# burmajam/delta_crdt_ex

Hardware: AMD Instinct MI355X
Metric: merged dots/sec for AWLWWMap delta join + Merkle diff keys/sec at 1–8 GPUs (higher is better)
Workload: dtype u64; 1 GPU; config2: 1M-key AWLWWMap full-state join of two replicas, 10% concurrent-write conflicts, per GPU (key-hash range shards); keys_per_gpu=1000000, rows_in_per_gpu=2000000, rows_out_per_gpu=1100011, parallelism=key-hash shards x1, rotate=4

## Files before the change

delta_crdt_ex_amd/csrc/api_engine.hip:

```cpp
#include <mutex>

#include <chrono>
#include <cstdarg>
#include <cstdio>
#include <cstdlib>

#include "dg_engine.h"

struct DevShare {
  int engines = 0;
  hipStream_t stream = nullptr;
};
std::mutex g_share_mu;
DevShare g_share[64];

hipStream_t shared_join_stream(dg_engine* e) {
  std::lock_guard<std::mutex> g(g_share_mu);
  DevShare& d = g_share[e->device & 63];
  if (d.engines < 2) return nullptr;
  if (!d.stream && hipStreamCreateWithFlags(&d.stream, hipStreamNonBlocking) != hipSuccess)
    d.stream = nullptr;
  return d.stream;
}

// ... 152 lines not shown
}

int check_store(const dg_store* s, const char* what) {
  if (!s) return fail(DG_E_INVAL, "%s: null store", what);
  if (s->n && (!s->key || !s->val || !s->ts || !s->node || !s->cnt))
    return fail(DG_E_INVAL, "%s: null column with n=%llu", what, (unsigned long long)s->n);
  return DG_OK;
}

int check_ctx(const dg_context* c, const char* what) {
  if (!c) return fail(DG_E_INVAL, "%s: null context", what);
  if (c->kind != DG_CTX_VV && c->kind != DG_CTX_DOTS)
    return fail(DG_E_INVAL, "%s: bad context kind %d", what, c->kind);
  if (c->n && (!c->node || !c->cnt)) return fail(DG_E_INVAL, "%s: null context column", what);
  return DG_OK;
}

bool pair_aligned(const void* k, const void* v, const void* t, const void* n, const void* c) {
  return !(((uintptr_t)k | (uintptr_t)v | (uintptr_t)t | (uintptr_t)c) & 15) && !((uintptr_t)n & 7);
}

int settle(dg_engine* e) {
  if (!e->pending.empty()) return dg_engine_sync(e);
  return DG_OK;
}

MerkleT merkle_of(const dg_merkle* t) {
  MerkleT m;
  m.depth = t->depth;
  m.sb = t->shard_bits;
  m.shard = t->shard;
  m.nodes = t->nodes;
  m.counts = t->counts;
  m.th = TermH{};
  if (t->terms) {
    m.th.nh = t->terms->node_hash;
    m.th.nn = t->terms->node_hash ? t->terms->n_nodes : 0;
    m.th.vid = t->terms->val_id;
    m.th.vh = t->terms->val_hash;
    m.th.nv = (t->terms->val_id && t->terms->val_hash) ? t->terms->n_vals : 0;
    m.th.on = 1;
  }
  m.starts = t->starts;
  return m;
}

int check_merkle(const dg_merkle* t, const char* what) {
  if (!t || !t->nodes) return fail(DG_E_INVAL, "%s: null tree", what);
  if (!t->counts || ((uintptr_t)t->counts & 15))
    return fail(DG_E_INVAL, "%s: the tree's counts must be a 16-byte aligned device array", what);
  if (t->depth < 1 || t->depth > 28) return fail(DG_E_INVAL, "%s: depth %u not in 1..28", what, t->depth);
  if (t->shard_bits > 16 || t->depth + t->shard_bits > 44)
    return fail(DG_E_INVAL, "%s: shard_bits %u (depth %u)", what, t->shard_bits, t->depth);
  if (t->shard_bits ? (t->shard >> t->shard_bits) != 0 : t->shard != 0)
    return fail(DG_E_INVAL, "%s: shard %llu >= 2^%u", what, (unsigned long long)t->shard, t->shard_bits);
  return DG_OK;
}

int tree_input_error(u32 bits, const char* what, const char* holds) {
  if (bits & MERKLE_ERR_SHARD) return fail(DG_E_INVAL, "%s: a key outside the tree's shard", what);
  if (bits & MERKLE_ERR_COUNT)
    return fail(DG_E_CAPACITY, "%s: a bucket %s more than 65535 rows (use a deeper tree)", what, holds);
  return DG_OK;
}

extern "C" {

int dg_abi_version(void) { return DG_ABI_VERSION; }

const char* dg_last_error(void) { return g_err.c_str(); }

int dg_engine_create(int device, void* hip_stream, dg_engine** out) {
  if (!out) return fail(DG_E_INVAL, "dg_engine_create: null out");
  *out = nullptr;
  int ndev = 0;
  HIP_TRY(hipGetDeviceCount(&ndev));
  if (device < 0 || device >= ndev)
    return fail(DG_E_INVAL, "dg_engine_create: device %d of %d", device, ndev);
  dg_engine* e = new dg_engine();
  e->device = device;
  {
    const char* v = getenv("DG_JOIN_WORKERS");
    if (v && atoi(v) > 0) e->join_workers = atoi(v);
    const char* m = getenv("DG_JOIN_MODE");
    if (m && m[0] == '2') e->join_mode = JOIN_TWO_PASS;
    const char* sp = getenv("DG_SPLICE");
    if (sp && sp[0] == '0') e->splice = false;
    const char* kd = getenv("DG_KD");
    if (kd && kd[0] == '0') e->kd = false;
    const char* am = getenv("DG_APPLY_MODE");
    if (am && strcmp(am, "fold") == 0) e->apply_mode = 1;
    if (am && strcmp(am, "onepass") == 0) e->apply_mode = 2;
    const char* tr = getenv("DG_TREE_REBUILD");
    if (tr && strcmp(tr, "always") == 0) e->tree_rebuild = dg_engine::TREE_ALWAYS;
    if (tr && strcmp(tr, "never") == 0) e->tree_rebuild = dg_engine::TREE_NEVER;
    if (tr && atoll(tr) > 0) e->tree_rebuild_div = (u64)atoll(tr);
  }
  int rc = set_device(e);
  if (rc != DG_OK) {
    delete e;
    return rc;
  }
  if (hip_stream) {
    e->stream = (hipStream_t)hip_stream;
  } else {
    if (hipStreamCreateWithFlags(&e->stream, hipStreamNonBlocking) != hipSuccess) {
      delete e;
      return fail(DG_E_DEVICE, "hipStreamCreate failed");
    }
    e->own_stream = true;
  }
  if (hipMalloc(&e->d_counts, 8 * sizeof(u64) + 16 * sizeof(u32)) != hipSuccess ||
      hipMalloc(&e->started, JOIN_MAX_GRID * sizeof(u32)) != hipSuccess ||
      hipHostMalloc(&e->h_counts, 16 * sizeof(u64), 0) != hipSuccess ||
      hipHostMalloc(&e->h_pub, 24 * sizeof(u64), hipHostMallocMapped | hipHostMallocCoherent) !=
          hipSuccess ||
      hipHostGetDevicePointer((void**)&e->d_pub, e->h_pub, 0) != hipSuccess) {
    dg_engine_destroy(e);
    return fail(DG_E_NOMEM, "dg_engine_create: allocation failed");
  }
  e->ticket = (u32*)(e->d_counts + 8);
  memset(e->h_pub, 0, 24 * sizeof(u64));
  if (hipMemsetAsync(e->d_counts, 0, 8 * sizeof(u64) + 16 * sizeof(u32), e->stream) != hipSuccess ||
      hipMemsetAsync(e->started, 0, JOIN_MAX_GRID * sizeof(u32), e->stream) != hipSuccess) {
    dg_engine_destroy(e);
    return fail(DG_E_DEVICE, "dg_engine_create: hipMemsetAsync failed");
  }
  rc = ensure_state(e, 4096);
  if (rc != DG_OK) {
    dg_engine_destroy(e);
    return rc;
  }
  if (hipEventCreateWithFlags(&e->ev_in, hipEventDisableTiming) != hipSuccess ||
      hipEventCreateWithFlags(&e->ev_out, hipEventDisableTiming) != hipSuccess) {
    dg_engine_destroy(e);
    return fail(DG_E_DEVICE, "dg_engine_create: hipEventCreate failed");
  }
  {
    std::lock_guard<std::mutex> g(g_share_mu);
    const int n = ++g_share[device & 63].engines;
    if (n == 2) hipDeviceSynchronize();
  }
  *out = e;
  return DG_OK;
}

int dg_engine_destroy(dg_engine* e) {
  if (!e) return DG_OK;
  hipSetDevice(e->device);
  if (e->stream) hipStreamSynchronize(e->stream);
  for (Buf* b : {&e->state, &e->tmp, &e->counts, &e->fold, &e->spl, &e->ubuf, &e->sml, &e->kdb, &e->kdz, &e->rpl,
                 &e->diff_bsum})
    if (b->p) hipFree(b->p);
  if (e->d_counts) hipFree(e->d_counts);
  if (e->h_counts) hipHostFree(e->h_counts);
  if (e->h_pub) hipHostFree(e->h_pub);
  if (e->started) hipFree(e->started);
  if (e->h_stage.p) hipHostFree(e->h_stage.p);
  if (e->h_cont.p) hipHostFree(e->h_cont.p);
  if (e->own_stream && e->stream) hipStreamDestroy(e->stream);
  if (e->ev_in || e->ev_out) {
    if (e->ev_in) hipEventDestroy(e->ev_in);
    if (e->ev_out) hipEventDestroy(e->ev_out);
    std::lock_guard<std::mutex> g(g_share_mu);
    DevShare& d = g_share[e->device & 63];
    if (e->ev_out && --d.engines == 0 && d.stream) {
// ... 58 lines not shown
```

delta_crdt_ex_amd/csrc/api_join.hip:

```cpp
#include "dg_engine.h"

int join2_enqueue(dg_engine* e, const dg_store* a, const dg_context* ca, const dg_store* b,
                  const dg_context* cb, const uint64_t* keys, uint64_t n_keys, dg_store* out,
                  dg_context* out_ctx, uint64_t* d_counts, void** chg, bool force_two_pass) {
  TRY(check_store(a, "dg_join2 a"));
  TRY(check_store(b, "dg_join2 b"));
  TRY(check_ctx(ca, "dg_join2 ca"));
  TRY(check_ctx(cb, "dg_join2 cb"));
  if (!out || !out_ctx || !d_counts) return fail(DG_E_INVAL, "dg_join2: null output");
  if (keys == nullptr && n_keys != 0) return fail(DG_E_INVAL, "dg_join2: keys NULL with n_keys>0");
  if (out->cap < a->n + b->n)
    return fail(DG_E_CAPACITY, "dg_join2: out cap %llu < %llu rows in", (unsigned long long)out->cap,
                (unsigned long long)(a->n + b->n));
  if (out_ctx->cap < ca->n + cb->n)
    return fail(DG_E_CAPACITY, "dg_join2: out_ctx cap %llu < %llu", (unsigned long long)out_ctx->cap,
                (unsigned long long)(ca->n + cb->n));
  if (a->n + b->n && (!out->key || !out->val || !out->ts || !out->node || !out->cnt))
    return fail(DG_E_INVAL, "dg_join2: null output column");
  TRY(set_device(e));
  const u64 tiles = join2_tiles(a->n, b->n), tiles_cap = join2_tiles_cap(a->n, b->n);
  Arena state;
  join_state_layout(state, tiles_cap);
  TRY(ensure_state(e, state.off / sizeof(u64)));
  const bool two_pass = (force_two_pass || e->join_mode == JOIN_TWO_PASS) && !chg;
  if (!two_pass) TRY(ensure_counts(e, tiles_cap));
  JoinScratch js;
  TRY(carve(e, &e->tmp, [&](Arena& m) {
    return join_layout(m, ctx_union_tmp_bytes(ca->n, cb->n),
                       two_pass ? measured([&](Arena& x) { pass_layout(x, tiles, JOIN_TILE); }) : 0,
                       chg ? measured([&](Arena& x) { chg_layout(x, tiles, JOIN_TILE); }) : 0);
  }, &js));
  if (chg) *chg = js.chg;
  Scan sc;
  TRY(next_scan(e, &sc));
  hipStream_t st = e->stream;
  hipStream_t ps = two_pass ? nullptr : shared_join_stream(e);
  if (ps) {
    HIP_TRY(hipEventRecord(e->ev_in, e->stream));
    HIP_TRY(hipStreamWaitEvent(ps, e->ev_in, 0));
    st = ps;
  }
  HIP_TRY(launch_join2(rows_of(a), ctx_of(ca), rows_of(b), ctx_of(cb), keys, keys ? n_keys : 0,
                       rows_out_of(out), out_ctx->node, out_ctx->cnt, js.ctx, js.pass,
                       two_pass ? JOIN_TWO_PASS : JOIN_SINGLE_PASS, sc, e->join_workers, d_counts, st, js.chg));
  if (ps) {
    HIP_TRY(hipEventRecord(e->ev_out, ps));
    HIP_TRY(hipStreamWaitEvent(e->stream, e->ev_out, 0));
  }
  out_ctx->kind = (ca->kind == DG_CTX_DOTS && cb->kind == DG_CTX_DOTS) ? DG_CTX_DOTS : DG_CTX_VV;
  return DG_OK;
}

bool splice_wanted(const dg_engine* e, const dg_store* a, const dg_store* b, const uint64_t* keys,
                   uint64_t n_keys, const dg_store* out) {
  return e->splice && keys && n_keys > 0 && (n_keys + b->n) * 8 <= a->n && out &&
         pair_aligned(a->key, a->val, a->ts, a->node, a->cnt) &&
         pair_aligned(out->key, out->val, out->ts, out->node, out->cnt);
}

int splice_take(dg_engine* e, const dg_store* a, const dg_store* b, const uint64_t* keys,
                uint64_t n_keys, u64 uctx_cap, Splice* w, bool* ok) {
  *ok = false;
  const u64 cap_k = std::min<u64>(a->n, 16 * n_keys + 4096);
  const u64 cap_e = cap_k + b->n;
  SpliceScratch s;
  TRY(carve(e, &e->spl, [&](Arena& m) { return splice_layout(m, cap_k, cap_e, n_keys, splice_tiles(a->n), uctx_cap); },
            &s));
  w->ak = s.ak;
  w->ed = s.ed;
  w->uctx = s.uctx;
  SpliceArgs& sp = w->sp;
  sp = SpliceArgs{};
  sp.a_lo = s.idx.a_lo;
  sp.a_off = s.idx.a_off;
  sp.end = s.idx.end;
  sp.shift = s.idx.shift;
  sp.gap = s.idx.gap;
  sp.tile_u0 = s.tile_u0;
  sp.moved = (u32*)(e->d_counts + SC_MOVED);
  TRY(ensure_state(e, take_tiles(n_keys) + 2));
  Scan sc;
  TRY(next_scan(e, &sc));
  static_assert(SC_BAD == SC_TAKEN + 1 && SC_MOVED == SC_TAKEN + 2, "zeroed as one range");
  HIP_TRY(hipMemsetAsync(e->d_counts + SC_TAKEN, 0, 3 * sizeof(u64), e->stream));
  u32* pre_len = nullptr;
  if (n_keys * 60 >= a->n) {
    pre_len = (u32*)sp.end;
    HIP_TRY(launch_splice_locate(rows_of(a), keys, n_keys, (u64*)sp.a_lo, pre_len, e->stream));
  }
  HIP_TRY(launch_take_keys(rows_of(a), keys, n_keys, rows_out_of(&w->ak), cap_k, sc,
                           e->d_counts + SC_TAKEN, e->stream, (u64*)sp.a_lo, (u64*)sp.a_off, pre_len));
  HIP_TRY(launch_splice_check(b->key, b->n, keys, n_keys, e->d_counts + SC_BAD, e->stream));
  TRY(read_counts(e));
  w->n_ak = e->h_counts[SC_TAKEN];
  if (e->h_counts[SC_BAD] != 0 || w->n_ak > cap_k) return DG_OK;
  w->ak.n = w->n_ak;
  sp.a = rows_of(a);
  sp.keys = keys;
  sp.nk = n_keys;
  sp.e = rows_of(&w->ed);
  sp.e.n = w->n_ak + b->n;
  sp.d_ne = e->d_counts + JC_ROWS;
  *ok = true;
  return DG_OK;
}

int splice_edit(dg_engine* e, Splice* w, const dg_context* ca, const dg_store* b,
                const dg_context* cb, const uint64_t* keys, uint64_t n_keys, dg_context* out_ctx,
                bool with_changes, uint64_t* changed, uint64_t cap) {
  void* chg = nullptr;
  TRY(join2_enqueue(e, &w->ak, ca, b, cb, keys, n_keys, &w->ed, out_ctx, e->d_counts,
                    with_changes ? &chg : nullptr));
  if (with_changes)
    HIP_TRY(launch_join2_changes(w->ak.n, b->n, chg, changed, cap, e->d_counts + JC_CHANGED, e->stream));
  HIP_TRY(launch_splice_index(w->sp, e->stream));
  return DG_OK;
}

static int splice_join(dg_engine* e, const dg_store* a, const dg_context* ca, const dg_store* b,
                       const dg_context* cb, const uint64_t* keys, uint64_t n_keys, dg_store* out,
                       dg_context* out_ctx, bool with_changes, uint64_t* changed, uint64_t cap,
                       uint64_t* n_changed, bool* done) {
  *done = false;
  TRY(check_store(a, "dg_join2 a"));
  TRY(check_store(b, "dg_join2 b"));
  TRY(check_ctx(ca, "dg_join2 ca"));
  TRY(check_ctx(cb, "dg_join2 cb"));
// ... 103 lines not shown
```

delta_crdt_ex_amd/csrc/dg_engine.h:

```cpp
#pragma once
#include <hip/hip_runtime.h>

#include <algorithm>
#include <cstring>
#include <string>
#include <vector>

#include "../../include/deltagpu.h"
#include "dg_arena.h"
#include "dg_hash.h"
#include "dg_launch.h"

using namespace dg;

struct Buf {
  void* p = nullptr;
  size_t cap = 0;
  template <class T>
  T* as() const { return (T*)p; }
};

struct dg_engine {
  int device = 0;
  hipStream_t stream = nullptr;
  bool own_stream = false;
  Buf state;
  u32* ticket = nullptr;
  Buf counts;
  u32* started = nullptr;
  Buf fold;
  bool splice = true;
  Buf spl;
  Buf ubuf;
  Buf sml;
  Buf kdb;
  Buf rpl;
  Buf kdz;
  bool kd = true;
  Buf diff_bsum;
  int diff_parity = 0;
  u32 epoch = 0;
  u64* d_counts = nullptr;
  u64* h_counts = nullptr;
  u64* h_pub = nullptr;
  u64* d_pub = nullptr;
  u64 pub_seq = 0;
  u32 h_ticket[16] = {};
  u32 last_err_bits = 0;
  Buf tmp;
  int join_mode = JOIN_SINGLE_PASS;
  int join_workers = 0;
  int apply_mode = 0;
  enum { TREE_BY_SHARE = 0, TREE_ALWAYS = 1, TREE_NEVER = 2 };
  int tree_rebuild = TREE_BY_SHARE;
  u64 tree_rebuild_div = 64;
  Buf h_stage;
  Buf h_cont;
  hipEvent_t ev_in = nullptr, ev_out = nullptr;
  struct Pending {
    int kind;
    dg_store a, b, out;
    dg_context ca, cb, out_ctx;
    const uint64_t* keys;
    uint64_t n_keys;
    uint64_t* d_counts;
    dg_merkle t;
    dg_merkle* tp;
  };
  std::vector<Pending> pending;
};


enum Ticket {
  TK_TILE = 0,
  TK_ERR = 1,
  TK_ORDER = 2,
  TK_INPUT = 3,
  TK_ABORT = 4,
  TK_UNUSED = 5,
  MERKLE_ARRIVE = 6,
  TAIL_ARRIVE = 7,
  KD_ARRIVE = 8,
  MUT_ARRIVE = 9,
  SPL_ARRIVE = 10,
  KD_ERR = 11,
  CONT_ARRIVE = 12,
};
constexpr int CONT_HOME = 18;

enum JoinCount {
  JC_ROWS = 0,
  JC_CTX = 1,
  JC_CHANGED = 2,
  SC_TAKEN = 3,
  SC_BAD = 4,
  SC_MOVED = 5,
};
enum HomeWord {
  HW_FLAGS = 0,
  HW_CTX = 3,
  HW_EDIT = 4,
  HW_TAKEN = 5,
  HW_MOVED = 6,
  HW_DKEYS = 7,
};
constexpr int TU_SHARDS = 8;
enum MutateCount {
  MC_KEYS = 0,
  MC_ROWS = 1,
  MC_SDOTS = 2,
};
enum MarkCount {
  MK_USED = 0,
  MK_UNKNOWN = 1,
};
constexpr int HC_KFOLD_FLAG = 10;

constexpr int RETRY_WORKERS = 32;

constexpr size_t MAX_PENDING = 4096;

hipStream_t shared_join_stream(dg_engine* e);

#pragma GCC visibility push(hidden)

extern thread_local std::string g_err;
int fail(int code, const char* fmt, ...);

#define HIP_TRY(expr)                                                                    \
  do {                                                                                   \
    hipError_t _e = (expr);                                                              \
    if (_e != hipSuccess)                                                                \
      return fail(DG_E_DEVICE, "%s failed: %s (%s:%d)", #expr, hipGetErrorString(_e),   \
                  __FILE__, __LINE__);                                                   \
// ... 117 lines not shown
```

delta_crdt_ex_amd/csrc/dg_jtile.h:

```cpp
#pragma once
#include "dg_ctxu.h"
#include "dg_launch.h"

namespace dg {

constexpr int JB = JOIN_BLOCK;
constexpr int JI = JOIN_ITEMS;
constexpr int JT = JOIN_TILE;
static_assert(JT % 2 == 0, "even tiles (balance_tiles keeps them even)");
constexpr int JS = JT + 5;
constexpr int VT = 64;

struct JoinArgs {
  Rows a, b;
  Ctx ca, cb;
  const u64* keys;
  u64 n_keys;
  const u64* splits;
  u64* ksplits;
  u64 ntiles;
  u64 jt;
  RowsOut out;
  Scan scan;
  u64* d_count;
  unsigned short* lists;
  u32* counts;
  u64* chg_tmp;
  u32* chg_cnt;
  u32* chg_wu;
  u64* chg_fk;
  u64* chg_lk;
  int fused;
  CtxUnionArgs cu;
};

constexpr int FUSE_IT = 4;
constexpr int CQ = (1024 + JB - 1) / JB;
static_assert((u64)CQ * JB + 1 <= JOIN_MAX_GRID, "start flags cover every join grid");
struct StreamKernels {
  void (*part)(JoinArgs);
  void (*fused)(JoinArgs);
};
#pragma GCC visibility push(hidden)
StreamKernels stream_kernels(bool fast, bool keyed, bool chg);
u64 resident_grid(const void* k);
hipError_t launch_stream(void (*kern)(JoinArgs), u64 grid, JoinArgs& p, hipStream_t st);
hipError_t launch_two_pass(JoinArgs& p, bool fast, bool keyed, void* pass_tmp, hipStream_t st);
#pragma GCC visibility pop

namespace {

constexpr int KS = 64;
struct KeySlice {
  const u64* lds;
  const u64* keys;
  u64 km;
};

__device__ __forceinline__ bool key_in(const KeySlice& ks, u64 x) {
  if (ks.lds) {
    const int km = (int)ks.km;
    int pos = 0;
#pragma unroll
    for (int step = KS; step >= 1; step >>= 1) {
      const int m = pos + step;
      const bool c = (m <= km) & (ks.lds[min(m, KS) - 1] < x);
      pos = c ? m : pos;
    }
    return (pos < km) & (ks.lds[min(pos, KS - 1)] == x);
  }
  return keyset_has(ks.keys, ks.km, x);
}

__device__ __forceinline__ bool fill_vv_tables(const Ctx& ca, const Ctx& cb, u64* tab_a, u64* tab_b) {
  bool far = false;
  for (u64 i = threadIdx.x; i < ca.n; i += JB) {
    const u32 nd = ca.node[i];
    if (nd < (u32)VT) tab_a[nd] = ca.cnt[i];
    far |= nd >= (u32)VT;
  }
  for (u64 i = threadIdx.x; i < cb.n; i += JB) {
    const u32 nd = cb.node[i];
    if (nd < (u32)VT) tab_b[nd] = cb.cnt[i];
    far |= nd >= (u32)VT;
  }
  return far;
}

struct Buf {
  alignas(16) u64 kv[JS][2];
  alignas(16) u64 tc[JS][2];
  u32 node[JS];
};

__device__ __forceinline__ u64 buf_key(const Buf& s, int x) { return s.kv[x][0]; }

__device__ __forceinline__ void buf_put(Buf& s, int x, u64 key, u64 val, i64 ts, u32 node, u64 cnt) {
  typedef u64 v2u64 __attribute__((ext_vector_type(2)));
  *(v2u64*)s.kv[x] = v2u64{key, val};
  *(v2u64*)s.tc[x] = v2u64{(u64)ts, cnt};
  s.node[x] = node;
}

__device__ __forceinline__ u64 slot_row(int x, int nat, u64 a0, u64 b0, u64 na, u64 nb,
                                        bool* from_b) {
  const bool in_a = x < nat + 2;
  const i64 g = in_a ? (i64)a0 - 1 + x : (i64)b0 - 1 + (x - (nat + 2));
  const bool fb = in_a ? na == 0 : nb != 0;
  const i64 last = (i64)(fb ? nb : na) - 1;
  *from_b = fb;
  return (u64)min(max(g, (i64)0), last);
}

constexpr int SLOTS = (JS + JB - 1) / JB;

// ... 153 lines not shown
```

delta_crdt_ex_amd/csrc/dg_launch.h:

```cpp
#pragma once
#include <hip/hip_runtime.h>
#include <stdint.h>

#include "dg_device.h"

namespace dg {

struct Scan {
  u64* state;
  u32* ticket;
  u32* err;
  u32 epoch;
  u32* counts;
  u32* started;
  u32* abort;
};

constexpr u64 JOIN_MAX_GRID = 2048;

#ifndef DG_JOIN_BLOCK
#define DG_JOIN_BLOCK 512
#endif
#ifndef DG_JOIN_ITEMS
#define DG_JOIN_ITEMS 2
#endif
constexpr int JOIN_BLOCK = DG_JOIN_BLOCK;
constexpr int JOIN_ITEMS = DG_JOIN_ITEMS;
constexpr int JOIN_TILE = JOIN_BLOCK * JOIN_ITEMS - 8;

inline u64 join2_tiles(u64 na, u64 nb) { return (na + nb + JOIN_TILE - 1) / JOIN_TILE; }
inline u64 join2_tiles_cap(u64 na, u64 nb) { return join2_tiles(na, nb) + JOIN_MAX_GRID; }
enum { JOIN_SINGLE_PASS = 0, JOIN_TWO_PASS = 1 };
hipError_t launch_join2(const Rows& a, const Ctx& ca, const Rows& b, const Ctx& cb,
                        const u64* keys, u64 n_keys, const RowsOut& out, u32* out_ctx_node,
                        u64* out_ctx_cnt, void* ctx_tmp, void* pass_tmp, int mode,
                        const Scan& scan, int workers, u64* d_counts, hipStream_t st,
                        void* chg_tmp = nullptr);
hipError_t launch_join2_changes(u64 na, u64 nb, void* chg_tmp, u64* out, u64 cap, u64* d_count,
                                hipStream_t st);
hipError_t launch_ctx_union(const Ctx& a, const Ctx& b, u32* out_node, u64* out_cnt,
                            u64* d_count, void* tmp, hipStream_t st);
inline size_t ctx_union_tmp_bytes(u64 na, u64 nb) {
  return (size_t)(na + nb) * 4 + (size_t)(na + nb) * 8 + (size_t)(na + nb + 1) * 4 + 64;
}

#ifndef DG_KFOLD_BLOCK
#define DG_KFOLD_BLOCK 1024
#endif
#ifndef DG_KFOLD_SCALE
#define DG_KFOLD_SCALE 0
#endif
constexpr int KFOLD_BLOCK = DG_KFOLD_BLOCK;
constexpr int KFOLD_CAP_S = 1024 >> DG_KFOLD_SCALE;
constexpr int KFOLD_CAP_D = 512 >> DG_KFOLD_SCALE;
constexpr int KFOLD_CAP_M = 512 >> DG_KFOLD_SCALE;
constexpr int KFOLD_MAX_K = 64;
constexpr int KNT = 1024;
constexpr u32 KF_PREP_FAIL = 1, KF_OVERFLOW = 2;
constexpr u64 KFOLD_FILL_SLICE = 2048;
constexpr u64 KFOLD_MEAN_S = 800 >> DG_KFOLD_SCALE, KFOLD_MEAN_D = 400 >> DG_KFOLD_SCALE,
              KFOLD_MEAN_M = 800 >> DG_KFOLD_SCALE, KFOLD_MEAN_U = 1200 >> DG_KFOLD_SCALE;
struct KRun {
  Rows rows;
  const u64* keys;
  u64 n_keys;
  Ctx ctx;
};
struct KFoldArgs {
  Rows s;
  Ctx c0;
  const KRun* runs;
  int k;
  u64 allmask;
  u64 T;
  u32 fill_p;
  u64* sstart;
  u32* dstart;
  u64* tabC;
  u64* tabP;
  RowsOut out;
  u32* out_ctx_node;
  u64* out_ctx_cnt;
  Scan scan;
  u64* d_counts;
  u32* flag;
  u64 dotsmask;
  u64* dset;
  u64 dset_mask;
  const u64* cflat;
  u64 dset_n;
};
constexpr u64 KF_EMPTY = ~0ull;
constexpr u64 KF_CNT_LIMIT = (1ull << 48) - 1;
hipError_t launch_kfold(const KFoldArgs& p, hipStream_t st);

#ifndef DG_TAKE_TILE
#define DG_TAKE_TILE 256
#endif
constexpr int TAKE_TILE = DG_TAKE_TILE;
inline u64 take_tiles(u64 n_keys) { return (n_keys + TAKE_TILE - 1) / TAKE_TILE; }
hipError_t launch_take_keys(const Rows& s, const u64* keys, u64 n_keys, const RowsOut& out,
                            u64 cap, const Scan& scan, u64* d_count, hipStream_t st,
                            u64* key_lo = nullptr, u64* key_off = nullptr,
                            const u32* pre_len = nullptr);

constexpr int KS_MAX_K = 64;
constexpr int KS_BLOCK = 256;
constexpr int KS_ITEMS = 4;
constexpr int KS_TILE = KS_BLOCK * KS_ITEMS;
inline u64 ks_tiles(u64 m) { return (m + KS_TILE - 1) / KS_TILE; }
struct KsSeg {
  const u64* keys;
  u64 off;
};
hipError_t launch_keysets_gather(const KsSeg* segs, int k, u64 m, u64* cat, uint8_t* set, u32* bad,
                                 hipStream_t st);
constexpr u64 KS_RANK_MAX = 1ull << 21;
hipError_t launch_keysets_rank(const KsSeg* segs, int k, u64 m, u64* skey, uint8_t* sset, u32* bad, hipStream_t st);
hipError_t launch_keysets_union(const u64* cat, const uint8_t* set, const u32* idx, u64 m, u64* ukeys_d,
                                u64* ukeys, u64* masks, u64 cap, const Scan& scan, u64* d_count,
// ... 400 lines not shown
```

delta_crdt_ex_amd/csrc/join.hip:

```cpp
#include <algorithm>

#include "dg_arena.h"
#include "dg_jsplit.h"
#include "dg_jtile.h"

namespace dg {

namespace {

constexpr int CB = 1024;

__global__ __launch_bounds__(CB) void ctx_union_kernel(CtxUnionArgs p) {
  __shared__ u32 s_wave[CB / WAVE + 1];
  ctx_union_block<CB>(p, s_wave);
}

__global__ __launch_bounds__(PB) void join2_partition_kernel(Rows A, Rows B, u64 ntiles, u64 jt,
                                                             u64* splits, CtxUnionArgs cu,
                                                             const u64* keys, u64 n_keys,
                                                             u64* ksplits) {
  if (blockIdx.x == 0) {
    __shared__ u32 s_wave[PB / WAVE + 1];
    ctx_union_block<PB>(cu, s_wave);
    return;
  }
  const u64 q = (u64)(blockIdx.x - 1) * (PB / WAVE) + (threadIdx.x >> 6);
  if (q > ntiles) return;
  const u64 d = min(q * jt, A.n + B.n);
  const u64 s = mp_split(A, B, d);
  if ((threadIdx.x & (WAVE - 1)) == 0) splits[q] = s;
  if (keys) {
    const u64 kq = key_split(A, B, keys, n_keys, d, s);
    if ((threadIdx.x & (WAVE - 1)) == 0) ksplits[q] = kq;
  }
}

}

static void balance_tiles(JoinArgs& p, u64 G) {
  const u64 total = p.a.n + p.b.n;
  if (G == 0 || p.ntiles <= G) return;
  const u64 k = (p.ntiles + G - 1) / G;
  const u64 jt = std::min<u64>(((total + k * G - 1) / (k * G) + 1) & ~1ull, JT);
  p.jt = jt;
  p.ntiles = (total + jt - 1) / jt;
}

hipError_t launch_join2(const Rows& a, const Ctx& ca, const Rows& b, const Ctx& cb,
                        const u64* keys, u64 n_keys, const RowsOut& out, u32* out_ctx_node,
                        u64* out_ctx_cnt, void* ctx_tmp, void* pass_tmp, int mode,
                        const Scan& scan, int workers, u64* d_counts, hipStream_t st,
                        void* chg_tmp) {
  JoinArgs p;
  p.a = a;
  p.b = b;
  p.ca = ca;
  p.cb = cb;
  p.keys = keys;
  p.n_keys = n_keys;
  p.ntiles = join2_tiles(a.n, b.n);
  p.jt = JT;
  JoinState js;
  auto place_splits = [&]() {
    Arena state(scan.state);
    js = join_state_layout(state, p.ntiles);
    p.splits = js.splits;
    p.ksplits = js.ksplits;
  };
  place_splits();
  const CtxUnionArgs cu = make_cu(ca, cb, out_ctx_node, out_ctx_cnt, d_counts + 1, ctx_tmp);
  p.out = out;
  p.scan = scan;
  p.d_count = d_counts;
  p.lists = nullptr;
  p.counts = nullptr;
  p.chg_tmp = nullptr;
  p.chg_cnt = p.chg_wu = nullptr;
  p.chg_fk = p.chg_lk = nullptr;
  if (chg_tmp) {
    Arena arena(chg_tmp);
    const ChgScratch l = chg_layout(arena, p.ntiles, JT);
    p.chg_tmp = l.ev;
    p.chg_cnt = l.cnt;
    p.chg_wu = l.wu;
    p.chg_fk = l.fk;
    p.chg_lk = l.lk;
  }
  if (p.ntiles == 0) {
    hipError_t e = hipMemsetAsync(d_counts, 0, sizeof(u64), st);
    if (e != hipSuccess) return e;
    hipLaunchKernelGGL(ctx_union_kernel, dim3(1), dim3(CB), 0, st, cu);
    return hipGetLastError();
  }
  const bool fast = ca.kind == 0 && cb.kind == 0;
  const bool keyed = keys != nullptr;
  p.fused = 0;
  p.cu = cu;
  const StreamKernels sk = stream_kernels(fast, keyed, chg_tmp != nullptr);
  auto kern = sk.part;
  auto kern_late = sk.fused;
  const bool stream = mode != JOIN_TWO_PASS || chg_tmp;
  u64 g = 0;
  if (stream) {
    g = workers > 0 ? (u64)workers : resident_grid((const void*)kern);
    g = std::min<u64>(std::min<u64>(p.ntiles, g), (u64)CQ * JB);
    static const bool no_fuse = [] {
      const char* v = getenv("DG_JOIN_FUSE");
      return v && v[0] == '0';
    }();
    const u64 gr = workers > 0 ? g + 1 : resident_grid((const void*)kern_late);
    const u64 gt = std::min<u64>(std::min<u64>(p.ntiles, gr - 1), (u64)CQ * JB);
    if (!no_fuse && gr >= 2 && p.ntiles <= (u64)FUSE_IT * gt) {
      if (!chg_tmp) balance_tiles(p, gt);
      place_splits();
      p.fused = 1;
      return launch_stream(kern_late, gt + 1, p, st);
    }
  }
  const u64 nb_part = (p.ntiles + 1 + (PB / WAVE) - 1) / (PB / WAVE);
  hipLaunchKernelGGL(join2_partition_kernel, dim3((unsigned)nb_part + 1), dim3(PB), 0, st, a, b,
                     p.ntiles, p.jt, js.splits, cu, keys, n_keys, js.ksplits);
  if (!stream) return launch_two_pass(p, fast, keyed, pass_tmp, st);
  return launch_stream(kern, g, p, st);
}

hipError_t launch_ctx_union(const Ctx& a, const Ctx& b, u32* out_node, u64* out_cnt,
                            u64* d_count, void* tmp, hipStream_t st) {
  CtxUnionArgs p = make_cu(a, b, out_node, out_cnt, d_count, tmp);
  hipLaunchKernelGGL(ctx_union_kernel, dim3(1), dim3(CB), 0, st, p);
  return hipGetLastError();
}

}
```

delta_crdt_ex_amd/csrc/join_stream.hip:

```cpp
#include <mutex>

#include "dg_jsplit.h"
#include "dg_jtile.h"

namespace dg {

namespace {

#ifdef DG_STAMPS
__device__ u64 g_join_stamps[65536 * 16];
#define JSTAMP(tile, k)                                                              \
  do {                                                                               \
    __syncthreads();                                                                 \
    __builtin_amdgcn_sched_barrier(0);                                               \
    if (threadIdx.x == 0 && (tile) < 65536) g_join_stamps[(tile) * 16 + (k)] =       \
        __builtin_amdgcn_s_memrealtime();                                            \
    __builtin_amdgcn_sched_barrier(0);                                               \
  } while (0)
#else
#define JSTAMP(tile, k) \
  do {                  \
  } while (0)
#endif


template <bool KEYED>
struct StreamLds {
  Buf buf[2];
  unsigned short comp[2][JT];
  u64 tab[2][VT];
  u64 kslice[2][KEYED ? KS : 1];
  u64 kspl[KEYED ? 2 * FUSE_IT : 1];
  u32 wave[JB / WAVE + 1];
  u64 red[2][2 * (JB / WAVE)];
  u64 spl[2 * FUSE_IT];
  u64 chk[JB / WAVE];
  int chf[JB / WAVE];
};

constexpr u32 CNT_BITS = 12;
static_assert(JT < (1 << CNT_BITS), "tile count must fit the granule's count field");

__device__ __forceinline__ void publish_count(u32* cs, u64 t, u32 epoch, u32 n) {
  __hip_atomic_store(cs + t, (epoch << CNT_BITS) | n, __ATOMIC_RELAXED, __HIP_MEMORY_SCOPE_AGENT);
}

struct StripeCounts {
  u32 v[CQ];
  bool ready;
};

__device__ __forceinline__ void stripe_load(const u32* cs, u64 base_t, u64 G, u64 ntiles, u32 epoch,
                                            StripeCounts& c) {
  c.ready = true;
#pragma unroll
  for (int q = 0; q < CQ; q++) {
    const u64 x = (u64)threadIdx.x + (u64)q * JB;
    const bool has = x < G && base_t + x < ntiles;
    c.v[q] = __hip_atomic_load(cs + base_t + (has ? x : 0), __ATOMIC_RELAXED,
                               __HIP_MEMORY_SCOPE_AGENT);
  }
}

constexpr u32 ABORT_POLLS = 1u << 13;

template <class T>
__device__ __forceinline__ T cold(const T* field) {
  return *(const volatile T*)field;
}

__device__ __forceinline__ const Scan* cold_scan() {
  return &((const JoinArgs*)__builtin_amdgcn_kernarg_segment_ptr())->scan;
}

__device__ __forceinline__ bool grid_check(u32 epoch, u32 spins, u64 need, const StripeCounts& c) {
  const Scan* sc = cold_scan();
  u32* abort = cold(&sc->abort);
  if (__hip_atomic_load(abort, __ATOMIC_RELAXED, __HIP_MEMORY_SCOPE_AGENT) == epoch) return true;
  if (spins <= ABORT_POLLS) return false;
  const u32* started = cold(&sc->started);
  bool absent = false;
#pragma unroll
  for (int q = 0; q < CQ; q++) {
    const u64 x = (u64)threadIdx.x + (u64)q * JB;
    if (x < need && (c.v[q] >> CNT_BITS) != epoch &&
        __hip_atomic_load(started + x, __ATOMIC_RELAXED, __HIP_MEMORY_SCOPE_AGENT) != epoch)
      absent = true;
  }
  if (!absent) return false;
  __hip_atomic_store(abort, cold(&sc->epoch), __ATOMIC_RELAXED, __HIP_MEMORY_SCOPE_AGENT);
  atomicOr(cold(&sc->err), 2u);
  return true;
}

__device__ __forceinline__ void stripe_sums(const u32* cs, u32 epoch, u32* err, u64 base_t,
                                            u64 G, u64 ntiles, u64 w, bool need_all,
                                            StripeCounts& c, u64* s_red, u64* below, u64* all) {
  const int tid = threadIdx.x;
#pragma unroll
  for (int q = 0; q < CQ; q++) {
    const u64 x = (u64)tid + (u64)q * JB;
    c.v[q] = x < G && base_t + x < ntiles ? c.v[q] : epoch << CNT_BITS;
  }
  const u64 need = need_all ? G : w;
  for (u32 spins = 0;; spins++) {
    bool ready = true;
#pragma unroll
    for (int q = 0; q < CQ; q++)
      ready &= (u64)tid + (u64)q * JB >= need || (c.v[q] >> CNT_BITS) == epoch;
    if (ready) break;
    if ((spins & 63) == 63 && grid_check(epoch, spins, need, c)) {
#pragma unroll
      for (int q = 0; q < CQ; q++)
        if ((c.v[q] >> CNT_BITS) != epoch) c.v[q] = epoch << CNT_BITS;
      break;
    }
    if (spins > (1u << 24)) {
      atomicOr(err, 1u);
      break;
    }
    __builtin_amdgcn_s_sleep(2);
    const u32* cs_poll = cold(&cold_scan()->counts);
#pragma unroll
    for (int q = 0; q < CQ; q++) {
      const u64 x = (u64)tid + (u64)q * JB;
      if (x < need && (c.v[q] >> CNT_BITS) != epoch)
        c.v[q] = __hip_atomic_load(cs_poll + base_t + x, __ATOMIC_RELAXED, __HIP_MEMORY_SCOPE_AGENT);
    }
  }
  u64 lo = 0, tot = 0;
#pragma unroll
  for (int q = 0; q < CQ; q++) {
    const u64 x = (u64)tid + (u64)q * JB;
    const u64 n = c.v[q] & ((1u << CNT_BITS) - 1);
    tot += n;
    lo += x < w ? n : 0;
  }
  lo = wave_sum_u32((u32)lo);
  tot = wave_sum_u32((u32)tot);
  constexpr int NW = JB / WAVE;
  if ((tid & (WAVE - 1)) == 0) {
    s_red[tid / WAVE] = lo;
    s_red[NW + tid / WAVE] = tot;
  }
  __syncthreads();
  lo = 0;
  tot = 0;
#pragma unroll
  for (int i = 0; i < NW; i++) {
    lo += s_red[i];
    tot += s_red[NW + i];
  }
  *below = lo;
  *all = tot;
}

template <bool KEYED>
__device__ __forceinline__ void write_tile(const JoinArgs& p, const StreamLds<KEYED>& s, int bi,
                                           u64 o0, u32 n) {
  const Buf& b = s.buf[bi];
  for (u32 q = threadIdx.x; q < n; q += JB) {
    const Row x = lds_row(b, s.comp[bi][q]);
    store_row_nt(p.out, o0 + q, x);
  }
}

template <bool FAST, bool KEYED, bool CHG, bool LATE>
__global__ __launch_bounds__(JB) __attribute__((amdgpu_waves_per_eu(4, 8))) void join2_stream_kernel(JoinArgs p) {
  __shared__ StreamLds<KEYED> s;
  const int tid = threadIdx.x;
  const u64 total = p.a.n + p.b.n, ntiles = p.ntiles, w = blockIdx.x;
  const u64 G = gridDim.x - (LATE ? 1 : 0);
  u32* cs = p.scan.counts;
  const u32 epoch = p.scan.epoch;
  const Rows& A = p.a;
  const Rows& B = p.b;
  if (tid == 0)
    __hip_atomic_store(cold(&cold_scan()->started) + w, epoch, __ATOMIC_RELAXED,
                       __HIP_MEMORY_SCOPE_AGENT);
  if (w < G) JSTAMP(w, 0);
  Staged r;
  u64 ga0 = 0, ga1 = 0;
  if (LATE) {
    if (w == G) {
      ctx_union_block<JB>(p.cu, s.wave);
      return;
    }
    {
      ga0 = split_guess(A.n, B.n, w * p.jt);
      ga1 = split_guess(A.n, B.n, min((w + 1) * p.jt, total));
      int gnat, gnbt;
      u64 gb0;
      tile_geom(w, p.jt, ga0, ga1, total, &gnat, &gnbt, &gb0);
      issue_tile(A, B, gnat, ga0, gb0, r);
    }
    for (int q = tid / WAVE; q < 2 * FUSE_IT; q += JB / WAVE) {
      const u64 tk = w + (u64)(q >> 1) * G;
      if (tk >= ntiles) break;
      const u64 d = min((tk + (q & 1)) * p.jt, total);
      const u64 g = split_guess(A.n, B.n, d);
      const u64 sp = guess_exact(A, B, d, g) ? g : mp_split(A, B, d);
      if ((tid & (WAVE - 1)) == 0) s.spl[q] = sp;
      if (KEYED) {
        const u64 kq = key_split(A, B, p.keys, p.n_keys, d, sp);
        if ((tid & (WAVE - 1)) == 0) s.kspl[q] = kq;
      }
    }
  }
  if (FAST)
    for (int x = tid; x < 2 * VT; x += JB) (&s.tab[0][0])[x] = 0;
  if (LATE) __syncthreads();
  if (w < G) JSTAMP(w, 8);
  auto split = [&](u64 tile, int k, int side) -> u64 {
    if (LATE) return s.spl[2 * k + side];
    return p.splits[tile + side];
  };
  auto kslice = [&](u64 tile, int k, u64* kl) -> u64 {
    u64 lo, hi;
    if (LATE) {
      lo = s.kspl[2 * k];
      hi = s.kspl[2 * k + 1];
    } else {
      lo = p.ksplits[tile];
      hi = p.ksplits[tile + 1];
    }
    *kl = lo;
    return min(hi + 1, p.n_keys) - lo;
  };
  u64 t = w;
  u64 a0 = split(t, 0, 0), a1 = split(t, 0, 1);
  constexpr bool AHEAD = !LATE && !KEYED;
  u64 sa0 = 0, sa1 = 0;
  auto splits_ahead = [&](u64 tile) {
    const u64 tq = min(tile, ntiles - 1);
    sa0 = p.splits[tq];
    sa1 = p.splits[tq + 1];
  };
  if (AHEAD) splits_ahead(t + G);
  int nat, nbt;
  u64 b0;
  tile_geom(t, p.jt, a0, a1, total, &nat, &nbt, &b0);
  if (!LATE || a0 != ga0 || a1 != ga1) issue_tile(A, B, nat, a0, b0, r);
  u64 kl = 0, km = 0, kk = 0;
  if (KEYED) {
    km = kslice(t, 0, &kl);
    if (km <= (u64)KS && (u64)tid < km) kk = p.keys[kl + tid];
  }
  __syncthreads();
  if (w < G) JSTAMP(w, 9);
  bool vv_far = false;
  if (FAST) {
    vv_far = fill_vv_tables(p.ca, p.cb, s.tab[0], s.tab[1]);
    if (LATE) vv_far = __syncthreads_or(vv_far);
  }
  u64 base = 0;
  u32 np = 0;
  for (int k = 0;; k++) {
    const int bi = k & 1;
    if (k > 0) JSTAMP(t, 0);
    JSTAMP(t, 1);
    commit_tile(r, s.buf[bi]);
    if (KEYED && km <= (u64)KS && (u64)tid < km) s.kslice[bi][tid] = kk;
    __syncthreads();
    JSTAMP(t, 2);
    const u64 tn = t + G;
    u64 a0n = 0, a1n = 0, b0n = 0, kln = 0, kmn = 0;
    int natn = 0, nbtn = 0;
    auto issue_next = [&]() {
      a0n = AHEAD ? sa0 : split(tn, k + 1, 0);
      a1n = AHEAD ? sa1 : split(tn, k + 1, 1);
      if (AHEAD) asm volatile("" : "+v"(a0n), "+v"(a1n) : : "memory");
      tile_geom(tn, p.jt, a0n, a1n, total, &natn, &nbtn, &b0n);
      issue_tile(A, B, natn, a0n, b0n, r);
      if (AHEAD) splits_ahead(tn + G);
      if (KEYED) {
        kmn = kslice(tn, k + 1, &kln);
        const u64 kls = ((u64)__builtin_amdgcn_readfirstlane((int)(kln >> 32)) << 32) |
                        (u32)__builtin_amdgcn_readfirstlane((int)kln);
        if (kmn <= (u64)KS && (u64)tid < kmn) kk = (p.keys + kls)[tid];
      }
    };
    if (tn < ntiles) issue_next();
    JSTAMP(t, 7);
    u32 keep, ev = 0;
    unsigned short src[JI];
    const KeySlice ks{KEYED && km <= (u64)KS ? s.kslice[bi] : nullptr, p.keys + kl, km};
    if (LATE && FAST && !vv_far)
      merge_items<FAST, KEYED, CHG, true>(p.ca, p.cb, s.tab[0], s.tab[1], ks, B.n, s.buf[bi], nat,
                                          nbt, a0, b0, keep, src, &ev);
    else
      merge_items<FAST, KEYED, CHG>(p.ca, p.cb, s.tab[0], s.tab[1], ks, B.n, s.buf[bi], nat, nbt, a0,
                                    b0, keep, src, &ev);
    JSTAMP(t, 3);
    u32 n;
    u32 pos = block_excl_scan1<JB>(__popc(keep), s.wave, &n);
#pragma unroll
    for (int q = 0; q < JI; q++)
      if (keep & (1u << q)) s.comp[bi][pos++] = src[q];
    if (tid == 0) publish_count(cs, t, epoch, n);
    StripeCounts sc;
    if (!CHG && k > 0) stripe_load(cs, t - G - w, G, ntiles, epoch, sc);
    __syncthreads();
    if (CHG) {
      const Buf& cb = s.buf[bi];
      const int ne = __popc(ev);
      u64 fkey = 0, lkey = 0;
      u32 diff = 0;
      bool seen = false;
#pragma unroll
      for (int q = 0; q < JI; q++)
        if (ev & (1u << q)) {
          const u64 k = buf_key(cb, src[q]);
          if (seen && k != lkey) diff++;
          if (!seen) fkey = k;
          lkey = k;
          seen = true;
        }
      const int lane = tid & (WAVE - 1), wv = tid / WAVE;
      const u32 mi = wave_incl_max(ne ? (u32)lane + 1 : 0u);
      const u32 mx = wave_prev(mi);
      const u64 pk = __shfl(lkey, mx > 0 ? (int)mx - 1 : 0, WAVE);
      const u32 ml = (u32)__builtin_amdgcn_readlane((int)mi, WAVE - 1);
      const u64 wk = __shfl(lkey, ml > 0 ? (int)ml - 1 : 0, WAVE);
      if (lane == WAVE - 1) {
        s.chf[wv] = (int)ml;
        s.chk[wv] = wk;
      }
      int pm = (int)mx;
      u64 pkey = pk;
      __syncthreads();
      if (pm == 0)
        for (int w2 = wv - 1; w2 >= 0; w2--)
          if (s.chf[w2] > 0) {
            pm = 1;
            pkey = s.chk[w2];
            break;
          }
      if (ne && pm > 0 && fkey != pkey) diff++;
      u32 tot2;
      const u32 sc2 = block_excl_scan1<JB>((diff << 16) | (u32)ne, s.wave, &tot2);
      const u32 n2 = tot2 & 0xffffu, p0 = sc2 & 0xffffu;
      u64* dst = p.chg_tmp + t * (u64)JT;
      u32 p2 = p0;
#pragma unroll
      for (int q = 0; q < JI; q++)
        if (ev & (1u << q)) dst[p2++] = buf_key(cb, src[q]);
      if (tid == 0) {
        p.chg_cnt[t] = n2;
        p.chg_wu[t] = tot2 >> 16;
      }
      if (ne && p0 == 0) p.chg_fk[t] = fkey;
      if (ne && p2 == n2) p.chg_lk[t] = lkey;
      if (k > 0) stripe_load(cs, t - G - w, G, ntiles, epoch, sc);
    }
    JSTAMP(t, 4);
    if (k > 0) {
      u64 below, all;
      stripe_sums(cs, epoch, p.scan.err, t - G - w, G, ntiles, w, true, sc, s.red[k & 1], &below,
                  &all);
      JSTAMP(t, 5);
      write_tile(p, s, bi ^ 1, base + below, np);
      base += all;
    }
    JSTAMP(t, 6);
    np = n;
    if (tn >= ntiles) {
      u64 below, all;
      StripeCounts last;
      stripe_load(cs, t - w, G, ntiles, epoch, last);
      stripe_sums(cs, epoch, p.scan.err, t - w, G, ntiles, w, false, last, s.red[(k + 1) & 1],
                  &below, &all);
      write_tile(p, s, bi, base + below, np);
      if (tid == 0 && t == ntiles - 1) p.d_count[0] = base + below + np;
      break;
    }
    t = tn;
    a0 = a0n;
    a1 = a1n;
    nat = natn;
    nbt = nbtn;
    b0 = b0n;
    kl = kln;
    km = kmn;
    __syncthreads();
  }
}

}

StreamKernels stream_kernels(bool fast, bool keyed, bool chg) {
  static void (*const kerns[2][2][2][2])(JoinArgs) = {
      {{{join2_stream_kernel<false, false, false, false>, join2_stream_kernel<false, false, false, true>},
        {join2_stream_kernel<false, false, true, false>, join2_stream_kernel<false, false, true, true>}},
       {{join2_stream_kernel<false, true, false, false>, join2_stream_kernel<false, true, false, true>},
        {join2_stream_kernel<false, true, true, false>, join2_stream_kernel<false, true, true, true>}}},
      {{{join2_stream_kernel<true, false, false, false>, join2_stream_kernel<true, false, false, true>},
        {join2_stream_kernel<true, false, true, false>, join2_stream_kernel<true, false, true, true>}},
       {{join2_stream_kernel<true, true, false, false>, join2_stream_kernel<true, true, false, true>},
        {join2_stream_kernel<true, true, true, false>, join2_stream_kernel<true, true, true, true>}}}};
  return {kerns[fast][keyed][chg][0], kerns[fast][keyed][chg][1]};
}

u64 resident_grid(const void* k) {
  struct Entry {
    const void* k;
    int dev;
    u64 n;
  };
  static Entry cache[32];
  static int used = 0;
  static std::mutex mu;
  int dev = 0;
  if (hipGetDevice(&dev) != hipSuccess) return 256;
  {
    std::lock_guard<std::mutex> g(mu);
    for (int i = 0; i < used; i++)
      if (cache[i].k == k && cache[i].dev == dev) return cache[i].n;
  }
  int per_cu = 0, cus = 0;
  if (hipDeviceGetAttribute(&cus, hipDeviceAttributeMultiprocessorCount, dev) != hipSuccess ||
      hipOccupancyMaxActiveBlocksPerMultiprocessor(&per_cu, k, JB, 0) != hipSuccess || per_cu <= 0 ||
      cus <= 0)
    return 256;
  const u64 n = (u64)per_cu * (u64)cus;
  std::lock_guard<std::mutex> g(mu);
  if (used < 32) cache[used++] = {k, dev, n};
  return n;
}

hipError_t launch_stream(void (*kern)(JoinArgs), u64 grid, JoinArgs& p, hipStream_t st) {
  static const bool coop = [] {
    const char* v = getenv("DG_JOIN_COOP");
    return v && v[0] == '1';
  }();
  if (!coop) {
    hipLaunchKernelGGL(kern, dim3((unsigned)grid), dim3(JB), 0, st, p);
    return hipGetLastError();
  }
  void* args[] = {&p};
  return hipLaunchCooperativeKernel((const void*)kern, dim3((unsigned)grid), dim3(JB), args, 0, st);
}

#ifdef DG_STAMPS
extern "C" int dg_debug_join_stamps(unsigned long long* host, size_t n) {
  if (n > 65536 * 16) n = 65536 * 16;
  return hipMemcpyFromSymbol(host, HIP_SYMBOL(g_join_stamps), n * 8) == hipSuccess ? 0 : -3;
}
#endif

}
```

Baseline: 60.35 billion merged dots/s.

## Use sliding-window stripe scan offsets and stagger upper join workers

```diff
diff --git a/delta_crdt_ex_amd/csrc/api_engine.hip b/delta_crdt_ex_amd/csrc/api_engine.hip
--- a/delta_crdt_ex_amd/csrc/api_engine.hip
+++ b/delta_crdt_ex_amd/csrc/api_engine.hip
@@ -258,6 +258,8 @@
   {
     const char* v = getenv("DG_JOIN_WORKERS");
     if (v && atoi(v) > 0) e->join_workers = atoi(v);
+    const char* sg = getenv("DG_JOIN_STAGGER");
+    if (sg && atoi(sg) > 0) e->join_stagger = atoi(sg) < 4096 ? atoi(sg) : 4096;
     const char* m = getenv("DG_JOIN_MODE");
     if (m && m[0] == '2') e->join_mode = JOIN_TWO_PASS;
     const char* sp = getenv("DG_SPLICE");
diff --git a/delta_crdt_ex_amd/csrc/api_join.hip b/delta_crdt_ex_amd/csrc/api_join.hip
--- a/delta_crdt_ex_amd/csrc/api_join.hip
+++ b/delta_crdt_ex_amd/csrc/api_join.hip
@@ -42,7 +42,8 @@
   }
   HIP_TRY(launch_join2(rows_of(a), ctx_of(ca), rows_of(b), ctx_of(cb), keys, keys ? n_keys : 0,
                        rows_out_of(out), out_ctx->node, out_ctx->cnt, js.ctx, js.pass,
-                       two_pass ? JOIN_TWO_PASS : JOIN_SINGLE_PASS, sc, e->join_workers, d_counts, st, js.chg));
+                       two_pass ? JOIN_TWO_PASS : JOIN_SINGLE_PASS, sc, e->join_workers, d_counts, st, js.chg,
+                       e->join_stagger));
   if (ps) {
     HIP_TRY(hipEventRecord(e->ev_out, ps));
     HIP_TRY(hipStreamWaitEvent(e->stream, e->ev_out, 0));
diff --git a/delta_crdt_ex_amd/csrc/dg_engine.h b/delta_crdt_ex_amd/csrc/dg_engine.h
--- a/delta_crdt_ex_amd/csrc/dg_engine.h
+++ b/delta_crdt_ex_amd/csrc/dg_engine.h
@@ -50,6 +50,7 @@
   Buf tmp;
   int join_mode = JOIN_SINGLE_PASS;
   int join_workers = 0;
+  int join_stagger = 0;
   int apply_mode = 0;
   enum { TREE_BY_SHARE = 0, TREE_ALWAYS = 1, TREE_NEVER = 2 };
   int tree_rebuild = TREE_BY_SHARE;
diff --git a/delta_crdt_ex_amd/csrc/dg_jstripe.h b/delta_crdt_ex_amd/csrc/dg_jstripe.h
--- /dev/null
+++ b/delta_crdt_ex_amd/csrc/dg_jstripe.h
@@ -0,0 +1,28 @@
+#pragma once
+#include <cstdint>
+
+#if defined(__HIPCC__) || defined(__CUDACC__)
+#define DG_JSTRIPE_HD __host__ __device__ __forceinline__
+#else
+#define DG_JSTRIPE_HD inline
+#endif
+
+namespace dg {
+
+struct StripeSlot {
+  uint64_t tile;
+  bool has, low;
+};
+
+DG_JSTRIPE_HD StripeSlot stripe_slot(uint64_t G, uint64_t t, uint64_t j) {
+  const bool has = j < G && t + j >= G;
+  StripeSlot s;
+  s.tile = has ? t + j - G : t;
+  s.has = has;
+  s.low = has && s.tile >= t - t % G;
+  return s;
+}
+
+DG_JSTRIPE_HD uint64_t stripe_position(uint64_t G, uint64_t tile) { return tile % G; }
+
+}
diff --git a/delta_crdt_ex_amd/csrc/dg_jtile.h b/delta_crdt_ex_amd/csrc/dg_jtile.h
--- a/delta_crdt_ex_amd/csrc/dg_jtile.h
+++ b/delta_crdt_ex_amd/csrc/dg_jtile.h
@@ -30,7 +30,7 @@
   u32* chg_wu;
   u64* chg_fk;
   u64* chg_lk;
-  int fused;
+  int stagger;
   CtxUnionArgs cu;
 };
 
diff --git a/delta_crdt_ex_amd/csrc/dg_launch.h b/delta_crdt_ex_amd/csrc/dg_launch.h
--- a/delta_crdt_ex_amd/csrc/dg_launch.h
+++ b/delta_crdt_ex_amd/csrc/dg_launch.h
@@ -35,7 +35,7 @@
                         const u64* keys, u64 n_keys, const RowsOut& out, u32* out_ctx_node,
                         u64* out_ctx_cnt, void* ctx_tmp, void* pass_tmp, int mode,
                         const Scan& scan, int workers, u64* d_counts, hipStream_t st,
-                        void* chg_tmp = nullptr);
+                        void* chg_tmp = nullptr, int stagger = 0);
 hipError_t launch_join2_changes(u64 na, u64 nb, void* chg_tmp, u64* out, u64 cap, u64* d_count,
                                 hipStream_t st);
 hipError_t launch_ctx_union(const Ctx& a, const Ctx& b, u32* out_node, u64* out_cnt,
diff --git a/delta_crdt_ex_amd/csrc/join.hip b/delta_crdt_ex_amd/csrc/join.hip
--- a/delta_crdt_ex_amd/csrc/join.hip
+++ b/delta_crdt_ex_amd/csrc/join.hip
@@ -50,7 +50,7 @@
                         const u64* keys, u64 n_keys, const RowsOut& out, u32* out_ctx_node,
                         u64* out_ctx_cnt, void* ctx_tmp, void* pass_tmp, int mode,
                         const Scan& scan, int workers, u64* d_counts, hipStream_t st,
-                        void* chg_tmp) {
+                        void* chg_tmp, int stagger) {
   JoinArgs p;
   p.a = a;
   p.b = b;
@@ -94,7 +94,7 @@
   }
   const bool fast = ca.kind == 0 && cb.kind == 0;
   const bool keyed = keys != nullptr;
-  p.fused = 0;
+  p.stagger = stagger;
   p.cu = cu;
   const StreamKernels sk = stream_kernels(fast, keyed, chg_tmp != nullptr);
   auto kern = sk.part;
@@ -113,7 +113,6 @@
     if (!no_fuse && gr >= 2 && p.ntiles <= (u64)FUSE_IT * gt) {
       if (!chg_tmp) balance_tiles(p, gt);
       place_splits();
-      p.fused = 1;
       return launch_stream(kern_late, gt + 1, p, st);
     }
   }
diff --git a/delta_crdt_ex_amd/csrc/join_stream.hip b/delta_crdt_ex_amd/csrc/join_stream.hip
--- a/delta_crdt_ex_amd/csrc/join_stream.hip
+++ b/delta_crdt_ex_amd/csrc/join_stream.hip
@@ -1,6 +1,7 @@
 #include <mutex>
 
 #include "dg_jsplit.h"
+#include "dg_jstripe.h"
 #include "dg_jtile.h"
 
 namespace dg {
@@ -17,9 +18,21 @@
         __builtin_amdgcn_s_memrealtime();                                            \
     __builtin_amdgcn_sched_barrier(0);                                               \
   } while (0)
+#define JSTAMP_PLACE(tile)                                                                 \
+  do {                                                                                     \
+    if (threadIdx.x == 0 && (tile) < 65536) {                                              \
+      g_join_stamps[(tile) * 16 + 10] =                                                    \
+          ((u64)__builtin_amdgcn_s_getreg((3 << 11) | 20) << 32) |                         \
+          (u64)__builtin_amdgcn_s_getreg((31 << 11) | 4);                                  \
+      g_join_stamps[(tile) * 16 + 11] = (u64)blockIdx.x + 1;                               \
+    }                                                                                      \
+  } while (0)
 #else
 #define JSTAMP(tile, k) \
   do {                  \
+  } while (0)
+#define JSTAMP_PLACE(tile) \
+  do {                     \
   } while (0)
 #endif
 
@@ -32,7 +45,7 @@
   u64 kslice[2][KEYED ? KS : 1];
   u64 kspl[KEYED ? 2 * FUSE_IT : 1];
   u32 wave[JB / WAVE + 1];
-  u64 red[2][2 * (JB / WAVE)];
+  u64 red[2][JB / WAVE];
   u64 spl[2 * FUSE_IT];
   u64 chk[JB / WAVE];
   int chf[JB / WAVE];
@@ -47,22 +60,18 @@
 
 struct StripeCounts {
   u32 v[CQ];
-  bool ready;
 };
 
-__device__ __forceinline__ void stripe_load(const u32* cs, u64 base_t, u64 G, u64 ntiles, u32 epoch,
-                                            StripeCounts& c) {
-  c.ready = true;
+__device__ __forceinline__ void stripe_load(const u32* cs, u64 t, u64 G, StripeCounts& c) {
 #pragma unroll
   for (int q = 0; q < CQ; q++) {
-    const u64 x = (u64)threadIdx.x + (u64)q * JB;
-    const bool has = x < G && base_t + x < ntiles;
-    c.v[q] = __hip_atomic_load(cs + base_t + (has ? x : 0), __ATOMIC_RELAXED,
-                               __HIP_MEMORY_SCOPE_AGENT);
+    const StripeSlot sl = stripe_slot(G, t, (u64)threadIdx.x + (u64)q * JB);
+    c.v[q] = __hip_atomic_load(cs + sl.tile, __ATOMIC_RELAXED, __HIP_MEMORY_SCOPE_AGENT);
   }
 }
 
 constexpr u32 ABORT_POLLS = 1u << 13;
+constexpr int STAGGER_SLEEP = 10;
 
 template <class T>
 __device__ __forceinline__ T cold(const T* field) {
@@ -73,7 +82,7 @@
   return &((const JoinArgs*)__builtin_amdgcn_kernarg_segment_ptr())->scan;
 }
 
-__device__ __forceinline__ bool grid_check(u32 epoch, u32 spins, u64 need, const StripeCounts& c) {
+__device__ __forceinline__ bool grid_check(u32 epoch, u32 spins, u64 t, u64 G, const StripeCounts& c) {
   const Scan* sc = cold_scan();
   u32* abort = cold(&sc->abort);
   if (__hip_atomic_load(abort, __ATOMIC_RELAXED, __HIP_MEMORY_SCOPE_AGENT) == epoch) return true;
@@ -82,9 +91,10 @@
   bool absent = false;
 #pragma unroll
   for (int q = 0; q < CQ; q++) {
-    const u64 x = (u64)threadIdx.x + (u64)q * JB;
-    if (x < need && (c.v[q] >> CNT_BITS) != epoch &&
-        __hip_atomic_load(started + x, __ATOMIC_RELAXED, __HIP_MEMORY_SCOPE_AGENT) != epoch)
+    if ((c.v[q] >> CNT_BITS) == epoch) continue;
+    const StripeSlot sl = stripe_slot(G, t, (u64)threadIdx.x + (u64)q * JB);
+    if (__hip_atomic_load(started + stripe_position(G, sl.tile), __ATOMIC_RELAXED,
+                          __HIP_MEMORY_SCOPE_AGENT) != epoch)
       absent = true;
   }
   if (!absent) return false;
@@ -93,23 +103,18 @@
   return true;
 }
 
-__device__ __forceinline__ void stripe_sums(const u32* cs, u32 epoch, u32* err, u64 base_t,
-                                            u64 G, u64 ntiles, u64 w, bool need_all,
-                                            StripeCounts& c, u64* s_red, u64* below, u64* all) {
+__device__ __forceinline__ u64 stripe_sums(u32 epoch, u32* err, u64 t, u64 G, StripeCounts& c,
+                                           u64* s_red) {
   const int tid = threadIdx.x;
 #pragma unroll
-  for (int q = 0; q < CQ; q++) {
-    const u64 x = (u64)tid + (u64)q * JB;
-    c.v[q] = x < G && base_t + x < ntiles ? c.v[q] : epoch << CNT_BITS;
-  }
-  const u64 need = need_all ? G : w;
+  for (int q = 0; q < CQ; q++)
+    if (!stripe_slot(G, t, (u64)tid + (u64)q * JB).has) c.v[q] = epoch << CNT_BITS;
   for (u32 spins = 0;; spins++) {
     bool ready = true;
 #pragma unroll
-    for (int q = 0; q < CQ; q++)
-      ready &= (u64)tid + (u64)q * JB >= need || (c.v[q] >> CNT_BITS) == epoch;
+    for (int q = 0; q < CQ; q++) ready &= (c.v[q] >> CNT_BITS) == epoch;
     if (ready) break;
-    if ((spins & 63) == 63 && grid_check(epoch, spins, need, c)) {
+    if ((spins & 63) == 63 && grid_check(epoch, spins, t, G, c)) {
 #pragma unroll
       for (int q = 0; q < CQ; q++)
         if ((c.v[q] >> CNT_BITS) != epoch) c.v[q] = epoch << CNT_BITS;
@@ -122,37 +127,22 @@
     __builtin_amdgcn_s_sleep(2);
     const u32* cs_poll = cold(&cold_scan()->counts);
 #pragma unroll
-    for (int q = 0; q < CQ; q++) {
-      const u64 x = (u64)tid + (u64)q * JB;
-      if (x < need && (c.v[q] >> CNT_BITS) != epoch)
-        c.v[q] = __hip_atomic_load(cs_poll + base_t + x, __ATOMIC_RELAXED, __HIP_MEMORY_SCOPE_AGENT);
-    }
-  }
-  u64 lo = 0, tot = 0;
-#pragma unroll
-  for (int q = 0; q < CQ; q++) {
-    const u64 x = (u64)tid + (u64)q * JB;
-    const u64 n = c.v[q] & ((1u << CNT_BITS) - 1);
-    tot += n;
-    lo += x < w ? n : 0;
-  }
-  lo = wave_sum_u32((u32)lo);
-  tot = wave_sum_u32((u32)tot);
+    for (int q = 0; q < CQ; q++)
+      if ((c.v[q] >> CNT_BITS) != epoch)
+        c.v[q] = __hip_atomic_load(cs_poll + stripe_slot(G, t, (u64)tid + (u64)q * JB).tile,
+                                   __ATOMIC_RELAXED, __HIP_MEMORY_SCOPE_AGENT);
+  }
+  u32 tot = 0;
+#pragma unroll
+  for (int q = 0; q < CQ; q++) tot += c.v[q] & ((1u << CNT_BITS) - 1);
+  tot = wave_sum_u32(tot);
   constexpr int NW = JB / WAVE;
-  if ((tid & (WAVE - 1)) == 0) {
-    s_red[tid / WAVE] = lo;
-    s_red[NW + tid / WAVE] = tot;
-  }
+  if ((tid & (WAVE - 1)) == 0) s_red[tid / WAVE] = tot;
   __syncthreads();
-  lo = 0;
-  tot = 0;
-#pragma unroll
-  for (int i = 0; i < NW; i++) {
-    lo += s_red[i];
-    tot += s_red[NW + i];
-  }
-  *below = lo;
-  *all = tot;
+  u32 sum = 0;
+#pragma unroll
+  for (int i = 0; i < NW; i++) sum += (u32)s_red[i];
+  return (u32)__builtin_amdgcn_readfirstlane((int)sum);
 }
 
 template <bool KEYED>
@@ -179,6 +169,7 @@
     __hip_atomic_store(cold(&cold_scan()->started) + w, epoch, __ATOMIC_RELAXED,
                        __HIP_MEMORY_SCOPE_AGENT);
   if (w < G) JSTAMP(w, 0);
+  if (w < G) JSTAMP_PLACE(w);
   Staged r;
   u64 ga0 = 0, ga1 = 0;
   if (LATE) {
@@ -253,10 +244,20 @@
     vv_far = fill_vv_tables(p.ca, p.cb, s.tab[0], s.tab[1]);
     if (LATE) vv_far = __syncthreads_or(vv_far);
   }
-  u64 base = 0;
+  if (2 * w >= G)
+    for (int i = cold(&((const JoinArgs*)__builtin_amdgcn_kernarg_segment_ptr())->stagger); i > 0; i--)
+      __builtin_amdgcn_s_sleep(STAGGER_SLEEP);
+  u64 off = 0;
   u32 np = 0;
+  const bool upper = 2 * w >= G;
   for (int k = 0;; k++) {
     const int bi = k & 1;
+    if (upper) {
+      if (k & 1)
+        __builtin_amdgcn_s_setprio(1);
+      else
+        __builtin_amdgcn_s_setprio(0);
+    }
     if (k > 0) JSTAMP(t, 0);
     JSTAMP(t, 1);
     commit_tile(r, s.buf[bi]);
@@ -299,7 +300,7 @@
       if (keep & (1u << q)) s.comp[bi][pos++] = src[q];
     if (tid == 0) publish_count(cs, t, epoch, n);
     StripeCounts sc;
-    if (!CHG && k > 0) stripe_load(cs, t - G - w, G, ntiles, epoch, sc);
+    if (!CHG && k > 0) stripe_load(cs, t - G, G, sc);
     __syncthreads();
     if (CHG) {
       const Buf& cb = s.buf[bi];
@@ -351,27 +352,22 @@
       }
       if (ne && p0 == 0) p.chg_fk[t] = fkey;
       if (ne && p2 == n2) p.chg_lk[t] = lkey;
-      if (k > 0) stripe_load(cs, t - G - w, G, ntiles, epoch, sc);
+      if (k > 0) stripe_load(cs, t - G, G, sc);
     }
     JSTAMP(t, 4);
     if (k > 0) {
-      u64 below, all;
-      stripe_sums(cs, epoch, p.scan.err, t - G - w, G, ntiles, w, true, sc, s.red[k & 1], &below,
-                  &all);
+      off += stripe_sums(epoch, p.scan.err, t - G, G, sc, s.red[k & 1]);
       JSTAMP(t, 5);
-      write_tile(p, s, bi ^ 1, base + below, np);
-      base += all;
+      write_tile(p, s, bi ^ 1, off, np);
     }
     JSTAMP(t, 6);
     np = n;
     if (tn >= ntiles) {
-      u64 below, all;
       StripeCounts last;
-      stripe_load(cs, t - w, G, ntiles, epoch, last);
-      stripe_sums(cs, epoch, p.scan.err, t - w, G, ntiles, w, false, last, s.red[(k + 1) & 1],
-                  &below, &all);
-      write_tile(p, s, bi, base + below, np);
-      if (tid == 0 && t == ntiles - 1) p.d_count[0] = base + below + np;
+      stripe_load(cs, t, G, last);
+      off += stripe_sums(epoch, p.scan.err, t, G, last, s.red[(k + 1) & 1]);
+      write_tile(p, s, bi, off, np);
+      if (tid == 0 && t == ntiles - 1) p.d_count[0] = off + np;
       break;
     }
     t = tn;
```

After: 67.66 billion merged dots/s (median of 6 runs). 12.1% higher.
